# sholtodouglas/RoboticsPlayroomPybullet

Measured on AMD Instinct MI355X. Metric: env-steps/sec at N=4096 parallel UR5PlayAbsRPY1Obj-v0 envs per MI355X, higher is better.
Workload: dtype f32

## Files before the change

### roboticsplayroompybullet_amd/csrc/rp_kernels.cuh

```cuda
#pragma once
#include <hip/hip_runtime.h>
#include <stdint.h>

#include "rp_device_model.h"
#include "rp_math.cuh"

#define NB_MAX (1 + RP_MAX_ARM + RP_MAX_FREE + RP_MAX_J1)
#define NVP 28
#define MAXC 21
#define MAXACT 64
#define MAXT 4
#define MAXROWC (3 * MAXC + MAXT)
static_assert(MAXACT <= 64 && NB_MAX <= 32, "a candidate record packs its pair index in 6 bits and its bodies in 5 bits each");
#define PM_MAX 11
#define PMC_HDR 4
#define PMC_PT 11
#define PMC_MAN (8 + 4 * PMC_PT)
#define PMC_MANIFOLDS (PMC_HDR + PM_MAX * PMC_MAN)
#define PMC_AX PMC_MANIFOLDS
#define PMC_AXN 16
#define PMC_FLOATS (PMC_MANIFOLDS + 8 * PMC_AXN)
#define RP_MAX_GROUPS 16
#define SORT_KEYS 64
#define SORT_REPS 8
// ... 208 lines not shown
__device__ __forceinline__ int lane_pos(const DevModel* m, int d) {
  if (d < m->n_arm) return d;
  const int e = d - m->n_arm, f6 = 6 * m->n_free;
  if (e >= f6) return LANE_J1 + (e - f6);
  const int f = e / 6, c = e - 6 * f;
  return f == m->drawer_free ? m->n_arm + c : LANE_FREE + 6 * f + c;
}
__device__ __forceinline__ int lane_dof(const DevModel* m, int l) {
  if (l < m->n_arm) return l;
  if (l < 16) return l - m->n_arm < 6 ? m->n_arm + 6 * m->drawer_free + (l - m->n_arm) : -1;
  if (l >= 32) return -1;
  if (l < LANE_FREE) return l - LANE_J1 < m->n_j1 ? m->n_arm + 6 * m->n_free + (l - LANE_J1) : -1;
  return l - LANE_FREE < 12 ? m->n_arm + (l - LANE_FREE) : -1;
}
#endif
__device__ __forceinline__ float clampf(float v, float lo, float hi) { return fminf(fmaxf(v, lo), hi); }
__device__ __forceinline__ float safe_inv(float d) { return d > 1e-9f ? 1.0f / d : 0.0f; }
__device__ __forceinline__ int uni(int v) { return __builtin_amdgcn_readfirstlane(v); }
__device__ __forceinline__ float unif(float v) { return __int_as_float(__builtin_amdgcn_readfirstlane(__float_as_int(v))); }
__device__ __forceinline__ float lane_read(float v, int src_lane_uniform) {
  return __int_as_float(__builtin_amdgcn_readlane(__float_as_int(v), src_lane_uniform));
}

__device__ __forceinline__ double readlane_d(double v, int src_lane_uniform) {
  int lo = __builtin_amdgcn_readlane(__double2loint(v), src_lane_uniform), hi = __builtin_amdgcn_readlane(__double2hiint(v), src_lane_uniform);
  return __hiloint2double(hi, lo);
}

template <int K>
__device__ __forceinline__ float bcast16(float v) {
  return __int_as_float(__builtin_amdgcn_update_dpp(0, __float_as_int(v), 0x150 + (K & 15), 0xF, 0xF, true));
}
template <int T> struct IdxC { static constexpr int v = T; };
template <int I, int N, class F>
__device__ __forceinline__ void static_for(F&& f) {
  if constexpr (I < N) { f(IdxC<I>{}); static_for<I + 1, N>(f); }
}

template <int D>
__device__ __forceinline__ float shr16(float v) {
  return __int_as_float(__builtin_amdgcn_update_dpp(__float_as_int(v), __float_as_int(v), 0x110 + D, 0xF, 0xF, false));
}

__device__ __forceinline__ float wave_sum32(float v) {
  int x = __float_as_int(v);
  v += __int_as_float(__builtin_amdgcn_update_dpp(0, x, 0xB1, 0xF, 0xF, true));
  x = __float_as_int(v);
  v += __int_as_float(__builtin_amdgcn_update_dpp(0, x, 0x4E, 0xF, 0xF, true));
  x = __float_as_int(v);
  v += __int_as_float(__builtin_amdgcn_update_dpp(0, x, 0x141, 0xF, 0xF, true));
  x = __float_as_int(v);
  v += __int_as_float(__builtin_amdgcn_update_dpp(0, x, 0x140, 0xF, 0xF, true));
  return lane_read(v, 0) + lane_read(v, 16);
}

__device__ __forceinline__ uint64_t splitmix64(uint64_t x) {
  x += 0x9E3779B97F4A7C15ULL;
  x = (x ^ (x >> 30)) * 0xBF58476D1CE4E5B9ULL;
  x = (x ^ (x >> 27)) * 0x94D049BB133111EBULL;
  return x ^ (x >> 31);
}
__device__ __forceinline__ float rng_uniform(uint64_t seed, uint32_t env, uint32_t counter) {
  uint64_t h = splitmix64(seed ^ splitmix64(((uint64_t)env << 32) | counter));
  return (float)(h >> 40) * (1.0f / 16777216.0f);
}

struct Xf { M3 R; V3 p; };

__device__ __forceinline__ Xf joint_compose(const DevModel* m, const Xf& P, int j, float q) {
  Xf r;
  M3 Rj = mul(P.R, ldm3(m->arm_jrot[j]));
  r.p = P.p + mulv(P.R, ld3(m->arm_jpos[j]));
  V3 ax = ld3(m->arm_axis[j]);
  if (m->arm_jtype[j] == 0) {
    r.R = mul(Rj, axis_angle(ax, q));
  } else {
    r.R = Rj;
    r.p = r.p + mulv(Rj, ax) * q;
  }
  return r;
}

template <class LDS>
__device__ __forceinline__ void fk_bodies(const DevModel* m, LDS& L, int lane) {
  float* T = L.cand;
  static_assert(2 * 12 * RP_MAX_ARM + 2 * RP_MAX_ARM <= CANDMAX * 8 && 2 * 12 * RP_MAX_ARM + 2 * RP_MAX_ARM <= (int)(sizeof(L.cand) / sizeof(float)), "fk scratch fits the candidate list");
  int* P = (int*)(T + 2 * 12 * RP_MAX_ARM);
  const int n = m->n_arm;
  Xf x; x.R = ident3(); x.p = mk3(0, 0, 0);
  int par = -1;
  if (lane < n) {
    M3 R0 = ldm3(m->arm_jrot[lane]);
    V3 p0 = ld3(m->arm_jpos[lane]), ax = ld3(m->arm_axis[lane]);
    float q = L.st[ST_Q + lane];
    x.R = R0; x.p = p0;
    if (m->arm_jtype[lane] == 0) x.R = mul(R0, axis_angle(ax, q));
    else x.p = p0 + mulv(R0, ax) * q;
    par = m->arm_parent[lane];
    if (par < 0) { M3 Rb = ldm3(m->base_rot); V3 pb = ld3(m->base_pos); x.p = pb + mulv(Rb, x.p); x.R = mul(Rb, x.R); }
  }
  for (int it = 0; __ballot(par >= 0) != 0ull; it++) {
    float* Tb = T + (it & 1) * 12 * RP_MAX_ARM;
    int* Pb = P + (it & 1) * RP_MAX_ARM;
    if (lane < n) { stm3(&Tb[12 * lane], x.R); st3(&Tb[12 * lane + 9], x.p); Pb[lane] = par; }
    WSYNC();
    if (par >= 0) {
      M3 Ra = ldm3(&Tb[12 * par]); V3 pa = ld3(&Tb[12 * par + 9]);
      x.p = pa + mulv(Ra, x.p); x.R = mul(Ra, x.R);
      par = Pb[par];
    }
  }
  if (lane < n) { stm3(&L.xR[9 * (lane + 1)], x.R); st3(&L.xp[3 * (lane + 1)], x.p); }
  if (lane < m->nbody && !(lane >= 1 && lane <= n)) {
    int b = lane;
    Xf y; y.R = ident3(); y.p = mk3(0, 0, 0);
    if (b > n && b <= n + m->n_free) {
      int k = b - 1 - n;
      const float* f = &L.st[ST_FREE + 13 * k];
      Q4 q = {f[3], f[4], f[5], f[6]};
      y.R = quat_to_m3(q); y.p = ld3(f);
    } else if (b > n + m->n_free) {
      int k = b - 1 - n - m->n_free;
      M3 R0 = ldm3(m->j1_rot[k]);
      V3 ax = ld3(m->j1_axis[k]);
      y.p = ld3(m->j1_pos[k]);
      float q = L.st[ST_JQ + k];
      if (m->j1_type[k] == 0) y.R = mul(R0, axis_angle(ax, q));
      else { y.R = R0; y.p = y.p + mulv(R0, ax) * q; }
    }
    stm3(&L.xR[9 * b], y.R); st3(&L.xp[3 * b], y.p);
  }
}

template <class LDS>
__device__ __forceinline__ void joint_subspaces(const DevModel* m, LDS& L, int lane) {
  if (lane == 0) st3(L.O, ld3(&L.xp[3 * m->site_body[RP_SITE_EE]]));
  WSYNC();
  if (lane < m->n_arm) {
    V3 O = ld3(L.O);
    M3 R = ldm3(&L.xR[9 * (1 + lane)]);
    V3 a = mulv(R, ld3(m->arm_axis[lane]));
    V6 S;
    if (m->arm_jtype[lane] == 0) { S.a = a; S.l = cross(ld3(&L.xp[3 * (1 + lane)]) - O, a); }
    else { S.a = mk3(0, 0, 0); S.l = a; }
    st6(&L.S[6 * lane], S);
  }
}

template <class LDS>
__device__ __forceinline__ Xf collider_xf(const DevModel* m, const LDS& L, int c) {
  int b = m->col_body[c];
  M3 Rb = ldm3(&L.xR[9 * b]);
  Xf x;
  x.R = mul(Rb, ldm3(m->col_rot[c]));
  x.p = ld3(&L.xp[3 * b]) + mulv(Rb, ld3(m->col_pos[c]));
  return x;
}

template <class LDS>
__device__ __forceinline__ void collider_aabbs(const DevModel* m, LDS& L, int lane) {
  if (lane < m->n_col) {
    Xf x = collider_xf(m, L, lane);
    V3 he = ld3(m->col_he[lane]);
    float e[3];
    for (int i = 0; i < 3; i++)
      e[i] = m->col_type[lane] == 0 ? fabsf(x.R.m[3 * i]) * he.x + fabsf(x.R.m[3 * i + 1]) * he.y + fabsf(x.R.m[3 * i + 2]) * he.z : he.x;
    *(float4*)&L.aabb[8 * lane] = make_float4(x.p.x - e[0], x.p.y - e[1], x.p.z - e[2], m->col_margin[lane]);
    *(float4*)&L.aabb[8 * lane + 4] = make_float4(x.p.x + e[0], x.p.y + e[1], x.p.z + e[2], 0.f);
  }
}

struct CPt { V3 p, n; float dist; };

__device__ __forceinline__ int sphere_box(V3 cs, float r, V3 cb, const M3& Rb, V3 hb, float margin, int sphere_is_b, CPt* out) {
  const V3 l = tmulv(Rb, cs - cb);
  V3 cl = l;
  bool inside = true;
  if (cl.x > hb.x) { cl.x = hb.x; inside = false; }
  if (cl.x < -hb.x) { cl.x = -hb.x; inside = false; }
  if (cl.y > hb.y) { cl.y = hb.y; inside = false; }
  if (cl.y < -hb.y) { cl.y = -hb.y; inside = false; }
  if (cl.z > hb.z) { cl.z = hb.z; inside = false; }
  if (cl.z < -hb.z) { cl.z = -hb.z; inside = false; }
  V3 nl; float dist;
  if (!inside) {
    const V3 df = cl - l;
    const float len = norm(df);
    dist = len - r;
    if (dist > margin) return 0;
    nl = df * (1.f / len);
  } else {
    const float px = hb.x - fabsf(l.x), py = hb.y - fabsf(l.y), pz = hb.z - fabsf(l.z);
    int k0 = 0; float best = 1e30f;
    if (px < best) { best = px; k0 = 0; }
    if (py < best) { best = py; k0 = 1; }
    if (pz < best) { best = pz; k0 = 2; }
    const float lk = k0 == 0 ? l.x : (k0 == 1 ? l.y : l.z), hk = k0 == 0 ? hb.x : (k0 == 1 ? hb.y : hb.z);
    const float nk = lk > 0.f ? -1.f : 1.f, ck = lk > 0.f ? hk : -hk;
    nl = mk3(k0 == 0 ? nk : 0.f, k0 == 1 ? nk : 0.f, k0 == 2 ? nk : 0.f);
    cl = mk3(k0 == 0 ? ck : cl.x, k0 == 1 ? ck : cl.y, k0 == 2 ? ck : cl.z);
    dist = -best - r;
  }
  const V3 nw = mulv(Rb, nl), pw = mulv(Rb, cl) + cb;
  out[0].p = pw - nw * (0.5f * dist);
  out[0].n = sphere_is_b ? nw : -nw;
  out[0].dist = dist;
  return 1;
}

#define NPG 8
#define NPG_SCRATCH 96
__device__ __forceinline__ V3 pick3(int i, V3 a, V3 b, V3 c) { return i == 0 ? a : (i == 1 ? b : c); }
__device__ __forceinline__ float pick1(int i, float a, float b, float c) { return i == 0 ? a : (i == 1 ? b : c); }

// ... 1406 lines not shown
  WSYNC();
}

#define SR_UNIT 0
#define SR_J1 1
#define SR_GEAR 2
#define SR_LIMIT 3

template <class LDS>
__device__ __forceinline__ void put_srow(LDS& L, int r, int type, int dofA, float sign, float rhs, float dinv, float lo, float hi, int dofB) {
  float* s = &L.srow[8 * r];
  s[0] = __int_as_float(type); s[1] = __int_as_float(dofA); s[2] = sign; s[3] = rhs; s[4] = dinv; s[5] = lo; s[6] = hi;
  s[7] = __int_as_float(dofB);
}

template <class LDS>
__device__ __forceinline__ int build_small_rows(const DevModel* m, LDS& L, int lane) {
  int n = m->n_arm, nr = 0;
  if (lane < m->n_j1) {
    int d = dof_j1(m, lane);
    float minv = m->j1_minv[lane], dinv = 1.f / minv;
    float des = m->j1_has_pos_motor[lane] ? K_KP * (m->j1_motor_target[lane] - L.st[ST_JQ + lane]) / K_DT : 0.f;
    float mx = m->j1_motor_maximp[lane];
    put_srow(L, lane, SR_J1, d, minv, (des - L.vstar[d]) * dinv, dinv, -mx, mx, 0);
  }
  nr = m->n_j1;
  {
    int i = lane >> 1, side = lane & 1;
    bool on = false; float pen = 0.f;
    if (lane < 2 * n && m->arm_limited[i]) {
      float q = L.st[ST_Q + i];
      pen = side == 0 ? q - m->arm_lower[i] : m->arm_upper[i] - q;
      on = m->spec_limits ? !(pen > K_LIMIT_ACTIVATION) : !(pen > 0.f);
    }
    unsigned long long mask = __ballot(on);
    if (on) {
      int r = nr + __popcll(mask & ((1ull << lane) - 1ull));
      float sgn = side == 0 ? 1.f : -1.f;
      float dinv = 1.f / L.Minv[i * 12 + i];
      float relv = sgn * L.vstar[i], pos_err = 0.f, vel_err = -relv;
      if (pen > 0.f) vel_err -= pen / K_DT; else pos_err = -pen * (m->spec_limits ? K_ERP : K_ERP_LIMIT) / K_DT;
      put_srow(L, r, SR_LIMIT, i, sgn, (pos_err + vel_err) * dinv, dinv, 0.f, K_LIMIT_MAXIMP, 0);
    }
    nr += __popcll(mask);
  }
  if (lane < n) {
    float dinv = 1.f / L.Minv[lane * 12 + lane];
    float mode = L.st[ST_MMODE + lane];
    float des = mode != 0.f ? K_KP * (L.st[ST_MTARGET + lane] - L.st[ST_Q + lane]) / K_DT : 0.f;
    float mx = L.st[ST_MMAXIMP + lane];
    put_srow(L, nr + lane, SR_UNIT, lane, 1.f, (des - L.vstar[lane]) * dinv, dinv, -mx, mx, 0);
  }
  nr += n;
  if (m->arm_type == RP_ARM_PANDA) {
    if (lane == 0) {
      int a = m->d9p, b = m->d10p;
      float ratio = -1.f;
      float diag = L.Minv[a * 12 + a] + 2.f * ratio * L.Minv[a * 12 + b] + ratio * ratio * L.Minv[b * 12 + b];
      float dinv = safe_inv(diag);
      float relv = L.vstar[a] + ratio * L.vstar[b];
      float pos_err = -(L.st[ST_Q + a] + ratio * L.st[ST_Q + b]) * 0.1f / K_DT;
      put_srow(L, nr, SR_GEAR, a, ratio, (pos_err - relv) * dinv, dinv, -50.f * K_DT, 50.f * K_DT, b);
    }
    nr += 1;
  }
  return nr;
}

template <class LDS>
__device__ __forceinline__ int tors_list(const DevModel* m, LDS& L, int lane, int ncon) {
  bool head = false; float spin = 0.f;
  if (lane < ncon) {
    const int a = L.cona[lane], b = L.conb[lane];
    head = lane == 0 || L.cona[lane - 1] != a || L.conb[lane - 1] != b;
    spin = m->col_spin[a] * m->col_friction[b] + m->col_spin[b] * m->col_friction[a];
  }
  const unsigned long long mk = __ballot(head && spin > 0.f);
  const int t = __popcll(mk & ((1ull << lane) - 1ull));
  if (head && spin > 0.f && t < MAXT) { L.torc[t] = lane; L.tors[t] = spin; }
  const int nt = __popcll(mk);
  return nt < MAXT ? nt : MAXT;
}

template <class LDS>
__device__ __forceinline__ void contact_rows(const DevModel* m, LDS& L, int lane, int c0, int nc, int nt) {
  const int n = m->n_arm;
  const int nrows = 3 * nc + nt;
  V3 O = ld3(L.O);
  for (int r = lane; r < nrows; r += 64) {
    int ci, dir;
    if (r < nc) { ci = c0 + r; dir = 0; }
    else if (r < nc + nt) { ci = L.torc[r - nc]; dir = 3; }
    else { ci = c0 + ((r - nc - nt) >> 1); dir = 1 + ((r - nc - nt) & 1); }
    V3 nrm = ld3(&L.conn[3 * ci]);
    const V3 pmid = ld3(&L.conp[3 * ci]);
    const V3 half = nrm * (0.5f * L.cond[ci]);
    V3 d = nrm;
    const bool tors = dir == 3;
    if (dir == 1 || dir == 2) {
      V3 t1, t2;
      if (fabsf(nrm.z) > 0.7071067811865475244f) {
        float a = nrm.y * nrm.y + nrm.z * nrm.z, k = 1.f / sqrtf(a);
        t1 = mk3(0.f, -nrm.z * k, nrm.y * k);
        t2 = mk3(a * k, -nrm.x * t1.z, nrm.x * t1.y);
      } else {
        float a = nrm.x * nrm.x + nrm.y * nrm.y, k = 1.f / sqrtf(a);
        t1 = mk3(-nrm.y * k, nrm.x * k, 0.f);
        t2 = mk3(-nrm.z * t1.y, nrm.z * t1.x, a * k);
      }
      d = dir == 1 ? t1 : t2;
    }
    float* J = &L.J[r * ROWW];
    float* B = &L.B[r * ROWW];
    for (int k = 0; k < ROWW; k++) { J[k] = 0.f; B[k] = 0.f; }
    bool has_arm = false;
    float diag = 0.f, relv = 0.f;
    int off0 = 64, off1 = 64;
    int bodyA = m->col_body[L.cona[ci]], bodyB = m->col_body[L.conb[ci]];
    bool any_arm = (bodyA >= 1 && bodyA <= n) || (bodyB >= 1 && bodyB <= n);
    int nother = 0;
    float Jr[RP_MAX_ARM];
#pragma unroll
    for (int k = 0; k < RP_MAX_ARM; k++) Jr[k] = 0.f;
    for (int side = 0; side < 2; side++) {
      int body = side == 0 ? bodyA : bodyB;
      float sign = side == 0 ? 1.f : -1.f;
      if (body == 0) continue;
      const V3 p = side == 0 ? pmid + half : pmid - half;
      if (body <= n) {
        V6 f; f.a = tors ? d : cross(p - O, d); f.l = tors ? mk3(0, 0, 0) : d;
        uint32_t anc = m->arm_anc[body - 1];
#pragma unroll
        for (int k = 0; k < RP_MAX_ARM; k++) {
          const float v = sign * dot6(ld6(&L.S[6 * k]), f);
          Jr[k] = (k < n && ((anc >> k) & 1u)) ? Jr[k] + v : Jr[k];
        }
        has_arm = true;
        continue;
      }
      int base = (any_arm || nother == 1) ? 12 : 0;
      nother++;
      if (body <= n + m->n_free) {
        int k = body - 1 - n, dd = dof_free(m, k);
        V3 rr = p - ld3(&L.st[ST_FREE + 13 * k]);
        V3 rxn = tors ? d : cross(rr, d);
        float im = 1.f / m->free_mass[k];
        M3 Ii = ldm3(&L.finv[9 * k]);
        V3 w = mulv(Ii, rxn);
        const V3 dl = tors ? mk3(0, 0, 0) : d;
        float jl[3] = {sign * dl.x, sign * dl.y, sign * dl.z}, ja[3] = {sign * rxn.x, sign * rxn.y, sign * rxn.z};
        float ba[3] = {sign * w.x, sign * w.y, sign * w.z};
        for (int i = 0; i < 3; i++) {
          J[base + i] = jl[i]; B[base + i] = jl[i] * im; J[base + 3 + i] = ja[i]; B[base + 3 + i] = ba[i];
          diag += jl[i] * jl[i] * im + ja[i] * ba[i];
          relv += jl[i] * L.vstar[dd + i] + ja[i] * L.vstar[dd + 3 + i];
        }
        if (base == 0) off0 = dd; else off1 = dd;
      } else {
        int k = body - 1 - n - m->n_free, dd = dof_j1(m, k);
        M3 R = ldm3(&L.xR[9 * body]);
        V3 a = mulv(R, ld3(m->j1_axis[k]));
        float j = tors ? (m->j1_type[k] == 1 ? 0.f : sign * dot(a, d)) : (m->j1_type[k] == 1 ? sign * dot(d, a) : sign * dot(a, cross(p - ld3(m->j1_pos[k]), d)));
        float minv = m->j1_minv[k];
        J[base] = j; B[base] = j * minv;
        diag += j * j * minv; relv += j * L.vstar[dd];
        if (base == 0) off0 = dd; else off1 = dd;
      }
    }
    if (has_arm) {
      off0 = 0;
#pragma unroll
      for (int k = 0; k < RP_MAX_ARM; k++) if (k < n) J[k] = Jr[k];
    }
    float* s = &L.rowS[4 * r];
    s[0] = diag; s[1] = relv; s[2] = dir == 0 ? 0.f : (tors ? L.tors[r - nc] : L.conmu[ci]); s[3] = __int_as_float(dir == 0 ? 0 : ci);
    float* t = &L.rowT[4 * r];
    t[0] = __int_as_float(has_arm ? 1 : 0); t[1] = dir == 0 ? 1e10f : 0.f; t[2] = __int_as_float(off0); t[3] = __int_as_float(off1);
  }
  WSYNC();
  for (int e = lane; e < nrows * n; e += 64) {
    int r = e / n, i = e - r * n;
    if (__float_as_int(L.rowT[4 * r]) != 0) {
      const float* J = &L.J[r * ROWW];
      const float* Mi = &L.Minv[i * 12];
      float b = 0.f;
#pragma unroll
      for (int k = 0; k < RP_MAX_ARM; k++) { const float t = Mi[k] * J[k]; b = k < n ? b + t : b; }
      L.B[r * ROWW + i] = b;
    }
  }
  WSYNC();
  for (int r = lane; r < nrows; r += 64) {
    float* s = &L.rowS[4 * r];
    float* t = &L.rowT[4 * r];
    float diag = s[0], relv = s[1];
    if (__float_as_int(t[0]) != 0) {
      const float* J = &L.J[r * ROWW];
      const float* B = &L.B[r * ROWW];
#pragma unroll
      for (int i = 0; i < RP_MAX_ARM; i++) { const float jb = J[i] * B[i], jv = J[i] * L.vstar[i]; diag = i < n ? diag + jb : diag; relv = i < n ? relv + jv : relv; }
    }
    float dinv, rhs, cfmr = 0.f;
    if (r < nc) {
      const int ci = c0 + r;
      float cfm = 0.f, erp = K_ERP;
      float s0 = m->col_stiff[L.cona[ci]], s1 = m->col_stiff[L.conb[ci]];
      if (s0 > 0.f || s1 > 0.f) {
        float d0 = s0 > 0.f ? m->col_damp[L.cona[ci]] : 0.1f, d1 = s1 > 0.f ? m->col_damp[L.conb[ci]] : 0.1f;
        if (!(s0 > 0.f)) s0 = 1e18f;
        if (!(s1 > 0.f)) s1 = 1e18f;
        float ks = 1.f / (1.f / s0 + 1.f / s1), kd = d0 + d1;
        cfm = 1.f / (K_DT * (K_DT * ks + kd));
        erp = (K_DT * ks) / (K_DT * ks + kd);
      }
      dinv = safe_inv(diag + cfm);
      cfmr = cfm * dinv;
      float pen = L.cond[ci] + K_SLOP, pos_err = 0.f, vel_err = -relv;
      if (pen > 0.f) vel_err -= pen / K_DT; else pos_err = -pen * erp / K_DT;
      rhs = (pos_err + vel_err) * dinv;
    } else { dinv = safe_inv(diag); rhs = -relv * dinv; }
    s[0] = rhs; s[1] = cfmr;
    t[0] = __int_as_float((__float_as_int(t[0]) != 0 && __float_as_int(t[3]) != 64) ? 1 : 0);
    float* Jw = &L.J[r * ROWW];
    for (int k = 0; k < ROWW; k++) Jw[k] *= dinv;
  }
}

__device__ __forceinline__ float pgs_update(float delta, float lam, float lo, float hi, float& lam_out) {
  float d = __builtin_amdgcn_fmed3f(delta, lo - lam, hi - lam);
  lam_out = lam + d;
  return d;
}

template <class LDS>
__device__ float solve_rows(const DevModel* m, LDS& L, int lane, int nsmall_, int ncon_, int nt_) {
  const int n = m->n_arm;
  const int nsmall = uni(nsmall_), nrc = uni(3 * ncon_ + nt_);
  float dv = 0.f;
  float lamS = 0.f, lamC0 = 0.f, lamC1 = 0.f;
  for (int it = 0; it < K_NITER; it++) {
    {
      for (int rr = 0; rr < nsmall; rr++) {
        const int r = (it & 1) ? rr : nsmall - 1 - rr;
        const float4 c0 = *(const float4*)&L.srow[8 * r], c1 = *(const float4*)&L.srow[8 * r + 4];
        const int type_ = uni(__float_as_int(c0.x)), dA = uni(__float_as_int(c0.y)), dB = uni(__float_as_int(c1.w));
        const int type = type_ == SR_LIMIT ? SR_UNIT : type_;
        const float sg = c0.z, jA = c1.x;
        float bl = 0.f;
        if (type == SR_J1) bl = lane == lane_pos(m, dA) ? sg : 0.f;
        else if (lane < n) bl = type == SR_UNIT ? sg * L.Minv[lane * 12 + dA] : L.Minv[lane * 12 + dA] + sg * L.Minv[lane * 12 + dB];
        float delta;
        if (type == SR_UNIT) delta = __fmaf_rn(-(sg * jA), lane_read(dv, dA), c0.w);
        else if (type == SR_J1) delta = __fmaf_rn(-jA, lane_read(dv, uni(lane_pos(m, dA))), c0.w);
        else { float pa = jA * lane_read(dv, dA); float pb = (sg * jA) * lane_read(dv, dB); float jdv = pa + pb; delta = c0.w - jdv; }
        float lam = lane_read(lamS, r), lnew;
        const float d = pgs_update(delta, lam, c1.y, c1.z, lnew);
        lamS = lane == r ? lnew : lamS;
        dv = fmaf(bl, d, dv);
      }
    }
    if (nrc > 0) {
      float4 sn = *(const float4*)&L.rowS[0], tn = *(const float4*)&L.rowT[0];
      float4 s2 = sn, t2 = tn;
      if (nrc > 1) { s2 = *(const float4*)&L.rowS[4]; t2 = *(const float4*)&L.rowT[4]; }
      float jn = 0.f, bn = 0.f;
      const int mydof = lane_dof(m, lane);
      {
        int i1 = mydof - __float_as_int(tn.w), i0 = mydof - __float_as_int(tn.z);
        int idx = (unsigned)i1 < 6u ? 12 + i1 : ((unsigned)i0 < 12u ? i0 : -1);
        if (idx >= 0 && mydof >= 0) { jn = L.J[idx]; bn = L.B[idx]; }
      }
      for (int r = 0; r < nrc; r++) {
        float jl = jn, bl = bn;
        float rhs = sn.x, cfmr = sn.y, mu = sn.z, lo_c = 0.f, hi_c = tn.y;
        int parent = uni(__float_as_int(sn.w));
// ... 901 lines not shown
    else if (nc == 6) { for (int rep = 0; rep < 4; rep++) qj = ik_coop<6>(m, tpos, tq, qj, 20, l16, live, &ik_capped, &ik_marginal); }
    else { for (int rep = 0; rep < 4; rep++) qj = ik_coop<7>(m, tpos, tq, qj, 20, l16, live, &ik_capped, &ik_marginal); }
  }
  if (!live) return;
  if (l16 < nd) {
    float t = clampf(qj, m->ll[l16], m->ul[l16]);
    t = clampf(t, q0 - m->inc[l16], q0 + m->inc[l16]);
    st[ST_MMODE + l16] = 1.f; st[ST_MTARGET + l16] = t; st[ST_MMAXIMP + l16] = 240.f * K_DT;
    if (target_poses) target_poses[(size_t)env * nd + l16] = t;
  }
  if (l16 == 0) {
    st[ST_STATUS] = __int_as_float((ik_capped ? 8 : 0) | (ik_marginal ? 16 : 0));
    float g = a8[m->n_action - 1];
    if (m->arm_type == RP_ARM_PANDA) {
      float amt = 0.04f - g / 25.f;
      int ds[2] = {m->d9p, m->d10p};
      for (int i = 0; i < 2; i++) { st[ST_MMODE + ds[i]] = 1.f; st[ST_MTARGET + ds[i]] = amt; st[ST_MMAXIMP + ds[i]] = 100.f * K_DT; }
    } else {
      float amt = g - 0.2f;
      float left = st[ST_Q + m->d18];
      int ds[6] = {m->d18, m->d20, m->d12, m->d15, m->d10, m->d13};
      float tg[6] = {amt * 0.055f, left, amt * 0.5f, amt * 0.5f, amt * 0.8f, amt * 0.8f};
      float fo[6] = {100.f, 1000.f, 100.f, 100.f, 100.f, 100.f};
      for (int i = 0; i < 6; i++) { st[ST_MMODE + ds[i]] = 1.f; st[ST_MTARGET + ds[i]] = tg[i]; st[ST_MMAXIMP + ds[i]] = fo[i] * K_DT; }
    }
  }
}

__global__ void __launch_bounds__(64) k_action(const DevModel* __restrict__ m, float* __restrict__ state, const float* __restrict__ action,
                                              float* __restrict__ target_poses, int env0, int N, const int* __restrict__ member) {
  action_body(m, state, action, target_poses, env0, N, member, blockIdx.x);
}

__device__ __forceinline__ void copy_out(float* __restrict__ dst, const float* src, int nfloat, int lane) {
  for (int i = lane * 4; i < nfloat; i += 256) *(float4*)(dst + i) = *(const float4*)(src + i);
}

#define NBJ 3
#define LBL_N NBJ
#define NLBL (LBL_N + MAXC)
#define GEAR_LANE 12
#define W3_HDR 0
#define W3_VSTAR 8
#define W3_MU 40
#define W3_MINV 72
#define W3_A 216
#define W3_GEAR (W3_A + 160)
#define W3_ZERO (W3_GEAR + 7)
#define W3_BJ (W3_GEAR + 8)
#define W3_ROWS (W3_BJ + 20)
#define W3_ROWT (W3_ROWS + 4 * MAXROWC)
#define W3_ROFF (W3_ROWT + 4 * MAXROWC)
#define W3_SLOT (W3_ROFF + 64)
#define W3_J (W3_SLOT + 64)
#define W3_B (W3_J + ROWREG)
#define W3_SROW (W3_B + ROWREG)
#define W3_FLOATS (W3_SROW + 4 + 8 * MAXSMALL)
#define STAGE_FLOATS (128 + 2 * ROWREG)
#define AOUT_FLOATS (160 + 8 + 20)
static_assert(W3_A % 4 == 0 && W3_ROWS % 4 == 0 && W3_ROFF % 4 == 0 && AOUT_FLOATS % 4 == 0, "16-byte copies");

#define HV_MAXC 14
#ifndef S4_SLOTS0
#define S4_SLOTS0 8
#endif
#ifndef S4_SLOTS1
#define S4_SLOTS1 8
#endif
__device__ __forceinline__ int hv_class(int nc, int nA, int nB, int nC) {
  const bool heavy = nC != 0 || nA > S4_SLOTS0 || nB > S4_SLOTS1;
  return !heavy ? 0 : (nc <= HV_MAXC ? 1 : 2);
}
#define PREP_THREADS 128
__device__ __forceinline__ void prep2_core(PrepLds& L, const DevModel* __restrict__ m, const float* __restrict__ state, float* __restrict__ ws, const int env, const int cenv,
                                           int* __restrict__ pair_tab, const int pair_idx, int* __restrict__ hv_cnt = nullptr, int* __restrict__ hv_list = nullptr, const int prep_flags = 0) {
  const int tid = threadIdx.x, wid = tid >> 6, lane = tid & 63;
  PCLK(6) PCLK(0) PCLK_ZERO(15) PCLK_ZERO(19) PCLK_ZERO(26) PCLK_ZERO(27) PCLK_ZERO(28) PCLK_ZERO(29) PCLK_ZERO(30) PCLK_ZERO(31)
  static_assert(RP_REC_FLOATS == PREP_THREADS, "one float of the record per thread");
  L.st[tid] = state[(size_t)env * RP_REC_FLOATS + tid];
  if (tid == 64) L.hdr[3] = pair_idx;
  if (tid == 64 && m->persist) L.hdr[2] = __float_as_int(m->pmcache[(size_t)cenv * PMC_FLOATS]);
  __syncthreads();
  PCLK(16)
  if (wid == 0) fk_bodies(m, L, lane);
  __syncthreads();
  PCLK(17)
  float* w = ws + (size_t)env * W3_FLOATS;
  if (wid == 0) {
    collider_aabbs(m, L, lane);
    WSYNC();
    PCLK(1)
    int ncon = collide<PrepLds>(m, L, lane, cenv, &L.hdr[2]);
    ncon = uni(ncon);
#ifdef RP_ABL_MAXCON
    if (ncon > RP_ABL_MAXCON) ncon = RP_ABL_MAXCON;
#endif
    if (lane == 0) L.hdr[0] = ncon;
    PCLK(2)
  } else {
    joint_subspaces(m, L, lane);
    PCLK(18)
    arm_dynamics(m, L, lane);
    unconstrained_velocities(m, L, lane);
    PCLK(3)
    int nsmall = build_small_rows(m, L, lane);
    nsmall = uni(nsmall);
    for (int i = lane; i < AOUT_FLOATS; i += 64) L.aout[i] = 0.f;
    if (lane < 2) L.amask[lane] = 0u;
    if (lane == 2) L.amask[2] = (unsigned)nsmall;
    WSYNC();
    bool gear = false;
    if (lane < nsmall) {
      const float* s = &L.srow[8 * lane];
      int type = __float_as_int(s[0]), dA = __float_as_int(s[1]);
      float sg = s[2], rhs = s[3], dinv = s[4], lo = s[5], hi = s[6];
      if (type == SR_UNIT) {
        L.aout[dA] = dinv; L.aout[16 + dA] = rhs; L.aout[32 + dA] = lo; L.aout[48 + dA] = hi;
      } else if (type == SR_LIMIT) {
        int pl = sg > 0.f ? 64 : 112;
        L.aout[pl + dA] = sg * rhs; L.aout[pl + 16 + dA] = sg * lo; L.aout[pl + 32 + dA] = sg * hi;
        atomicOr(&L.amask[sg > 0.f ? 0 : 1], 1u << dA);
      } else if (type == SR_J1) {
        int k = lane;
        if (k < NBJ) { float* bq = &L.aout[168]; bq[k] = dinv; bq[4 + k] = rhs; bq[8 + k] = lo; bq[12 + k] = hi; bq[16 + k] = sg; }
      } else {
        float* g = &L.aout[160];
        g[0] = s[1]; g[1] = s[7]; g[2] = sg; g[3] = dinv; g[4] = rhs; g[5] = lo; g[6] = hi;
        gear = true;
      }
    }
    const bool anygear = __ballot(gear) != 0ull;
    if (lane == 0) L.hdr[1] = anygear ? 1 : 0;
    WSYNC();
    if (lane < 32) w[W3_VSTAR + lane] = L.vstar[lane];
    copy_out(w + W3_MINV, L.Minv, 144, lane);
    copy_out(w + W3_A, L.aout, AOUT_FLOATS, lane);
  }
  __syncthreads();
  const int ncon = L.hdr[0];
  int tid_j = threadIdx.x;
  asm volatile("" : "+v"(tid_j));
  const int wid_j = tid_j >> 6;
  if (wid_j == 0) {
    const int lane = tid_j & 63;
    float* w = ws + (size_t)env * W3_FLOATS;
    const int cls = lane < ncon ? L.conk[lane] : 3;
    const unsigned long long mB = __ballot(cls == 0), mA = __ballot(cls == 1), mC = __ballot(cls == 2);
    const unsigned long long lower = (1ull << lane) - 1ull;
    L.slot[lane] = -1;
    L.roff[lane] = 0;
    const int nt = tors_list(m, L, lane, ncon);
    WSYNC();
    if (cls == 0) L.slot[__popcll(mB & lower)] = lane;
    else if (cls == 1) L.slot[21 + __popcll(mA & lower)] = lane;
    else if (cls == 2) L.slot[42 + __popcll(mC & lower)] = lane;
    bool tors_done = nt == 0;
    for (int c0 = 0; c0 < ncon || !tors_done; c0 += PREP_CH) {
      const int nc = max(0, min(PREP_CH, ncon - c0));
      const int ntl = (!tors_done && c0 + PREP_CH >= ncon && 3 * nc + nt <= 3 * PREP_CH) ? nt : 0;
      contact_rows(m, L, lane, c0, nc, ntl);
      WSYNC();
      auto global_row = [&](int lr) { return lr < nc ? c0 + lr : (lr < nc + ntl ? 3 * ncon + (lr - nc) : ncon + 2 * c0 + (lr - nc - ntl)); };
      for (int e = lane; e < (3 * nc + ntl) * ROWW; e += 64) {
        const int lr = e / ROWW, k = e - lr * ROWW;
        const int gr = global_row(lr);
        w[W3_J + gr * ROWW + k] = L.J[e]; w[W3_B + gr * ROWW + k] = L.B[e];
      }
      for (int e = lane; e < (3 * nc + ntl) * 4; e += 64) {
        const int lr = e >> 2, k = e & 3;
        const int gr = global_row(lr);
        float v = L.rowS[e];
        if (k == 3 && lr >= nc && lr < nc + ntl) {
          const int c = L.torc[lr - nc], kc = L.conk[c];
          const unsigned long long mk = kc == 1 ? mA : (kc == 2 ? mC : mB);
          v = __int_as_float(c | (kc << 8) | (__popcll(mk & ((1ull << c) - 1ull)) << 12));
        }
        w[W3_ROWS + gr * 4 + k] = v; w[W3_ROWT + gr * 4 + k] = L.rowT[e];
      }
      if (lane < 3 * nc + ntl && !(lane >= nc && lane < nc + ntl)) {
        const int gr = global_row(lane);
        L.roff[gr] = __float_as_int(L.rowT[4 * lane + 2]) | (__float_as_int(L.rowT[4 * lane + 3]) << 8);
      }
      if (ntl > 0) tors_done = true;
      WSYNC();
    }
    PCLK(4)
    if (lane == 0) {
      int nj = m->n_j1 < NBJ ? m->n_j1 : NBJ;
      w[W3_HDR] = __int_as_float((int)L.amask[0]); w[W3_HDR + 1] = __int_as_float((int)L.amask[1]);
      w[W3_HDR + 2] = __int_as_float(nj); w[W3_HDR + 3] = __int_as_float(ncon);
      w[W3_HDR + 4] = __int_as_float(__popcll(mA)); w[W3_HDR + 5] = __int_as_float(__popcll(mB));
      w[W3_HDR + 6] = __int_as_float(L.hdr[1] | (nt << 8)); w[W3_HDR + 7] = __int_as_float(__popcll(mC));
      if (hv_list != nullptr && (hv_class(ncon, __popcll(mA), __popcll(mB), __popcll(mC)) != 0 || (prep_flags & 1))) hv_list[atomicAdd(hv_cnt, 1)] = env | (ncon << 24);
    }
    if (lane < 32) w[W3_MU + lane] = lane < ncon ? L.conmu[lane] : 0.f;
    copy_out(w + W3_ROFF, (const float*)L.roff, 64, lane);
    copy_out(w + W3_SLOT, (const float*)L.slot, 64, lane);
  } else {
    if ((tid_j & 63) == 0) pair_tab[L.hdr[3]] = env | (ncon << 24);
    if (prep_flags & 1) {
      const int lane = tid_j & 63;
      float* w = ws + (size_t)env * W3_FLOATS;
      const int nsm = (int)L.amask[2];
      if (lane == 0) w[W3_SROW] = __int_as_float(nsm);
      for (int i = lane; i < 8 * nsm; i += 64) w[W3_SROW + 4 + i] = L.srow[i];
    }
  }
  PCLK(5) PCLK(7)
}
__device__ __forceinline__ void prep2_body(const DevModel* __restrict__ m, const float* __restrict__ state, float* __restrict__ ws, int env0, int N,
                                           const int* __restrict__ sort_cnt, int* __restrict__ sort_cnt_next, const int* __restrict__ sort_slot, int* __restrict__ pair_env,
                                           const int* __restrict__ member, const int bid, const int* __restrict__ cache_env = nullptr, int* __restrict__ hv_cnt = nullptr, int* __restrict__ hv_cnt_next = nullptr,
                                           int* __restrict__ hv_list = nullptr, const int prep_flags = 0) {
  __shared__ PrepLds L;
  const int tid = threadIdx.x, wid = tid >> 6, lane = tid & 63;
  int env = env0 + bid;
  if (env >= N) return;
  if (member) env = member[env];
  if (bid == 0) {
    for (int i = tid; i < SORT_BINS; i += PREP_THREADS) sort_cnt_next[i] = 0;
    if (tid == 0 && hv_cnt_next) *hv_cnt_next = 0;
  }
  int pair_place = 0;
  if (wid == 1) {
    const int my_slot = sort_slot[env];
    int cnt8[8];
#pragma unroll
    for (int t = 0; t < 8; t++) cnt8[t] = sort_cnt[8 * lane + t];
    const int mybin = my_slot >> SORT_RANK_BITS;
    int above = 0;
#pragma unroll
    for (int t = 0; t < 8; t++) above += (8 * lane + t > mybin) ? cnt8[t] : 0;
#pragma unroll
    for (int d = 32; d >= 1; d >>= 1) above += __shfl_xor(above, d);
    pair_place = above + (my_slot & SORT_RANK_MASK);
  }
  prep2_core(L, m, state, ws, env, cache_env ? cache_env[env] : env, pair_env, env0 + pair_place, hv_cnt, hv_list ? hv_list + env0 : nullptr, prep_flags);
}
#define PREP2_ARGS const DevModel* __restrict__ m, const float* __restrict__ state, float* __restrict__ ws, int env0, int N, \
                   const int* __restrict__ sort_cnt, int* __restrict__ sort_cnt_next, const int* __restrict__ sort_slot, int* __restrict__ pair_env, \
                   const int* __restrict__ member
#define HV_ARGS int* __restrict__ hv_cnt, int* __restrict__ hv_cnt_next, int* __restrict__ hv_list, int prep_flags
__global__ void __launch_bounds__(PREP_THREADS, RP_PREP_WAVES) k_prep2(PREP2_ARGS, HV_ARGS) { prep2_body(m, state, ws, env0, N, sort_cnt, sort_cnt_next, sort_slot, pair_env, member, blockIdx.x, nullptr, hv_cnt, hv_cnt_next, hv_list, prep_flags); }
__global__ void __launch_bounds__(PREP_THREADS, RP_PREP_WAVES) k_settle_prep(PREP2_ARGS, const int* __restrict__ cache_env, int prep_flags) { prep2_body(m, state, ws, env0, N, sort_cnt, sort_cnt_next, sort_slot, pair_env, member, blockIdx.x, cache_env, nullptr, nullptr, nullptr, prep_flags); }
__global__ void __launch_bounds__(PREP_THREADS, RP_PREP_WAVES) k_action_prep(const DevModel* __restrict__ m, float* __restrict__ state, float* __restrict__ ws, int env0, int N,
                                                                   const int* __restrict__ sort_cnt, int* __restrict__ sort_cnt_next, const int* __restrict__ sort_slot,
                                                                   int* __restrict__ pair_env, const int* __restrict__ member, const float* __restrict__ action,
                                                                   float* __restrict__ target_poses, int nab, HV_ARGS) {
  if ((int)blockIdx.x < nab) {
    __builtin_amdgcn_s_setprio(3);
    action_body(m, state, action, target_poses, env0, N, member, blockIdx.x);
  }
  else prep2_body(m, state, ws, env0, N, sort_cnt, sort_cnt_next, sort_slot, pair_env, member, blockIdx.x - nab, nullptr, hv_cnt, hv_cnt_next, hv_list, prep_flags);
}


typedef float f16v __attribute__((ext_vector_type(16)));
__device__ __forceinline__ float row16_sum(float v) {
  int x = __float_as_int(v);
  v += __int_as_float(__builtin_amdgcn_update_dpp(0, x, 0xB1, 0xF, 0xF, true));
  x = __float_as_int(v);
  v += __int_as_float(__builtin_amdgcn_update_dpp(0, x, 0x4E, 0xF, 0xF, true));
  x = __float_as_int(v);
  v += __int_as_float(__builtin_amdgcn_update_dpp(0, x, 0x141, 0xF, 0xF, true));
  x = __float_as_int(v);
  v += __int_as_float(__builtin_amdgcn_update_dpp(0, x, 0x140, 0xF, 0xF, true));
  return v;
}
__device__ __forceinline__ float fold_rows(float v) {
  unsigned u = __float_as_uint(v);
  auto sw = __builtin_amdgcn_permlane16_swap(u, u, false, false);
  return __uint_as_float(sw[0]) + __uint_as_float(sw[1]);
}
struct Plane { float rhs, lo, hi, lam, dacc, loP, hiP; };
struct PlaneN : Plane { float cfm, rhsE; };
#define PLANE_FENCE4(a, b, c, d) asm volatile("s_nop 1" : "+v"((a).loP), "+v"((a).hiP), "+v"((b).loP), "+v"((b).hiP), "+v"((c).loP), "+v"((c).hiP), "+v"((d).loP), "+v"((d).hiP))
#define PLANE_FENCE_N(a, b, c) asm volatile("s_nop 1" : "+v"((a).loP), "+v"((a).hiP), "+v"((b).rhsE), "+v"((c).rhsE))
__device__ __forceinline__ void plane_begin(Plane& p) { p.loP = p.lo - p.lam; p.hiP = p.hi - p.lam; p.dacc = 0.f; }
__device__ __forceinline__ void plane_end(Plane& p) { p.lam += p.dacc; }
__device__ __forceinline__ void nplane_begin(PlaneN& p) { p.loP = p.lo - p.lam; p.hiP = p.hi - p.lam; p.dacc = 0.f; p.rhsE = __fmaf_rn(-p.lam, p.cfm, p.rhs); }
__device__ __forceinline__ void fplane_begin(Plane& p, float lim, float tot) {
  const bool on = tot > 0.f;
  p.loP = on ? (0.f - lim) - p.lam : 0.f; p.hiP = on ? (0.f + lim) - p.lam : 0.f; p.dacc = 0.f;
}

#define DPP_ALL " row_mask:0xf bank_mask:0xf bound_ctrl:1\n"

template <int I>
// ... 1466 lines not shown
```

Measured before the change: 2.136 million.

## Spread contact-row build and body FK across all block wavefronts

The prep kernel's contact Jacobian row construction, previously run by wavefront 0 alone while other waves idled, now runs across all PREP_THREADS threads, with block-wide barriers in place of wave syncs. Forward kinematics is split so wave 0 handles the arm chain while the other waves compute free and single-joint bodies at the same time. This aims to shorten the serial critical path per environment, at the cost of more __syncthreads barriers and a shared torsion count passed through LDS.

```diff
diff --git a/roboticsplayroompybullet_amd/csrc/rp_kernels.cuh b/roboticsplayroompybullet_amd/csrc/rp_kernels.cuh
--- a/roboticsplayroompybullet_amd/csrc/rp_kernels.cuh
+++ b/roboticsplayroompybullet_amd/csrc/rp_kernels.cuh
@@ -314,7 +314,7 @@
 }
 
 template <class LDS>
-__device__ __forceinline__ void fk_bodies(const DevModel* m, LDS& L, int lane) {
+__device__ __forceinline__ void fk_arm_links(const DevModel* m, LDS& L, int lane) {
   float* T = L.cand;
   static_assert(2 * 12 * RP_MAX_ARM + 2 * RP_MAX_ARM <= CANDMAX * 8 && 2 * 12 * RP_MAX_ARM + 2 * RP_MAX_ARM <= (int)(sizeof(L.cand) / sizeof(float)), "fk scratch fits the candidate list");
   int* P = (int*)(T + 2 * 12 * RP_MAX_ARM);
@@ -343,6 +343,10 @@
     }
   }
   if (lane < n) { stm3(&L.xR[9 * (lane + 1)], x.R); st3(&L.xp[3 * (lane + 1)], x.p); }
+}
+template <class LDS>
+__device__ __forceinline__ void fk_other_bodies(const DevModel* m, LDS& L, int lane) {
+  const int n = m->n_arm;
   if (lane < m->nbody && !(lane >= 1 && lane <= n)) {
     int b = lane;
     Xf y; y.R = ident3(); y.p = mk3(0, 0, 0);
@@ -362,6 +366,11 @@
     }
     stm3(&L.xR[9 * b], y.R); st3(&L.xp[3 * b], y.p);
   }
+}
+template <class LDS>
+__device__ __forceinline__ void fk_bodies(const DevModel* m, LDS& L, int lane) {
+  fk_arm_links(m, L, lane);
+  fk_other_bodies(m, L, lane);
 }
 
 template <class LDS>
@@ -1934,12 +1943,16 @@
   return nt < MAXT ? nt : MAXT;
 }
 
-template <class LDS>
+template <int NTHR>
+__device__ __forceinline__ void rows_sync() {
+  if constexpr (NTHR == 64) WSYNC(); else __syncthreads();
+}
+template <class LDS, int NTHR = 64>
 __device__ __forceinline__ void contact_rows(const DevModel* m, LDS& L, int lane, int c0, int nc, int nt) {
   const int n = m->n_arm;
   const int nrows = 3 * nc + nt;
   V3 O = ld3(L.O);
-  for (int r = lane; r < nrows; r += 64) {
+  for (int r = lane; r < nrows; r += NTHR) {
     int ci, dir;
     if (r < nc) { ci = c0 + r; dir = 0; }
     else if (r < nc + nt) { ci = L.torc[r - nc]; dir = 3; }
@@ -2029,8 +2042,8 @@
     float* t = &L.rowT[4 * r];
     t[0] = __int_as_float(has_arm ? 1 : 0); t[1] = dir == 0 ? 1e10f : 0.f; t[2] = __int_as_float(off0); t[3] = __int_as_float(off1);
   }
-  WSYNC();
-  for (int e = lane; e < nrows * n; e += 64) {
+  rows_sync<NTHR>();
+  for (int e = lane; e < nrows * n; e += NTHR) {
     int r = e / n, i = e - r * n;
     if (__float_as_int(L.rowT[4 * r]) != 0) {
       const float* J = &L.J[r * ROWW];
@@ -2041,8 +2054,8 @@
       L.B[r * ROWW + i] = b;
     }
   }
-  WSYNC();
-  for (int r = lane; r < nrows; r += 64) {
+  rows_sync<NTHR>();
+  for (int r = lane; r < nrows; r += NTHR) {
     float* s = &L.rowS[4 * r];
     float* t = &L.rowT[4 * r];
     float diag = s[0], relv = s[1];
@@ -3110,7 +3123,8 @@
   if (tid == 64 && m->persist) L.hdr[2] = __float_as_int(m->pmcache[(size_t)cenv * PMC_FLOATS]);
   __syncthreads();
   PCLK(16)
-  if (wid == 0) fk_bodies(m, L, lane);
+  if (wid == 0) fk_arm_links(m, L, lane);
+  else fk_other_bodies(m, L, lane);
   __syncthreads();
   PCLK(17)
   float* w = ws + (size_t)env * W3_FLOATS;
@@ -3168,70 +3182,72 @@
   const int ncon = L.hdr[0];
   int tid_j = threadIdx.x;
   asm volatile("" : "+v"(tid_j));
-  const int wid_j = tid_j >> 6;
+  const int wid_j = tid_j >> 6, lane_j = tid_j & 63;
+  float* wr = ws + (size_t)env * W3_FLOATS;
+  const int cls = lane_j < ncon ? L.conk[lane_j] : 3;
+  const unsigned long long mB = __ballot(cls == 0), mA = __ballot(cls == 1), mC = __ballot(cls == 2);
   if (wid_j == 0) {
-    const int lane = tid_j & 63;
-    float* w = ws + (size_t)env * W3_FLOATS;
-    const int cls = lane < ncon ? L.conk[lane] : 3;
-    const unsigned long long mB = __ballot(cls == 0), mA = __ballot(cls == 1), mC = __ballot(cls == 2);
-    const unsigned long long lower = (1ull << lane) - 1ull;
-    L.slot[lane] = -1;
-    L.roff[lane] = 0;
-    const int nt = tors_list(m, L, lane, ncon);
+    const unsigned long long lower = (1ull << lane_j) - 1ull;
+    L.slot[lane_j] = -1;
+    L.roff[lane_j] = 0;
+    const int nt = tors_list(m, L, lane_j, ncon);
+    if (lane_j == 0) L.hdr[2] = nt;
     WSYNC();
-    if (cls == 0) L.slot[__popcll(mB & lower)] = lane;
-    else if (cls == 1) L.slot[21 + __popcll(mA & lower)] = lane;
-    else if (cls == 2) L.slot[42 + __popcll(mC & lower)] = lane;
-    bool tors_done = nt == 0;
-    for (int c0 = 0; c0 < ncon || !tors_done; c0 += PREP_CH) {
-      const int nc = max(0, min(PREP_CH, ncon - c0));
-      const int ntl = (!tors_done && c0 + PREP_CH >= ncon && 3 * nc + nt <= 3 * PREP_CH) ? nt : 0;
-      contact_rows(m, L, lane, c0, nc, ntl);
-      WSYNC();
-      auto global_row = [&](int lr) { return lr < nc ? c0 + lr : (lr < nc + ntl ? 3 * ncon + (lr - nc) : ncon + 2 * c0 + (lr - nc - ntl)); };
-      for (int e = lane; e < (3 * nc + ntl) * ROWW; e += 64) {
-        const int lr = e / ROWW, k = e - lr * ROWW;
-        const int gr = global_row(lr);
-        w[W3_J + gr * ROWW + k] = L.J[e]; w[W3_B + gr * ROWW + k] = L.B[e];
-      }
-      for (int e = lane; e < (3 * nc + ntl) * 4; e += 64) {
-        const int lr = e >> 2, k = e & 3;
-        const int gr = global_row(lr);
-        float v = L.rowS[e];
-        if (k == 3 && lr >= nc && lr < nc + ntl) {
-          const int c = L.torc[lr - nc], kc = L.conk[c];
-          const unsigned long long mk = kc == 1 ? mA : (kc == 2 ? mC : mB);
-          v = __int_as_float(c | (kc << 8) | (__popcll(mk & ((1ull << c) - 1ull)) << 12));
-        }
-        w[W3_ROWS + gr * 4 + k] = v; w[W3_ROWT + gr * 4 + k] = L.rowT[e];
-      }
-      if (lane < 3 * nc + ntl && !(lane >= nc && lane < nc + ntl)) {
-        const int gr = global_row(lane);
-        L.roff[gr] = __float_as_int(L.rowT[4 * lane + 2]) | (__float_as_int(L.rowT[4 * lane + 3]) << 8);
-      }
-      if (ntl > 0) tors_done = true;
-      WSYNC();
-    }
-    PCLK(4)
-    if (lane == 0) {
+    if (cls == 0) L.slot[__popcll(mB & lower)] = lane_j;
+    else if (cls == 1) L.slot[21 + __popcll(mA & lower)] = lane_j;
+    else if (cls == 2) L.slot[42 + __popcll(mC & lower)] = lane_j;
+  }
+  __syncthreads();
+  const int nt = uni(L.hdr[2]);
+  bool tors_done = nt == 0;
+  for (int c0 = 0; c0 < ncon || !tors_done; c0 += PREP_CH) {
+    const int nc = max(0, min(PREP_CH, ncon - c0));
+    const int ntl = (!tors_done && c0 + PREP_CH >= ncon && 3 * nc + nt <= 3 * PREP_CH) ? nt : 0;
+    contact_rows<PrepLds, PREP_THREADS>(m, L, tid_j, c0, nc, ntl);
+    __syncthreads();
+    auto global_row = [&](int lr) { return lr < nc ? c0 + lr : (lr < nc + ntl ? 3 * ncon + (lr - nc) : ncon + 2 * c0 + (lr - nc - ntl)); };
+    for (int e = tid_j; e < (3 * nc + ntl) * ROWW; e += PREP_THREADS) {
+      const int lr = e / ROWW, k = e - lr * ROWW;
+      const int gr = global_row(lr);
+      wr[W3_J + gr * ROWW + k] = L.J[e]; wr[W3_B + gr * ROWW + k] = L.B[e];
+    }
+    for (int e = tid_j; e < (3 * nc + ntl) * 4; e += PREP_THREADS) {
+      const int lr = e >> 2, k = e & 3;
+      const int gr = global_row(lr);
+      float v = L.rowS[e];
+      if (k == 3 && lr >= nc && lr < nc + ntl) {
+        const int c = L.torc[lr - nc], kc = L.conk[c];
+        const unsigned long long mk = kc == 1 ? mA : (kc == 2 ? mC : mB);
+        v = __int_as_float(c | (kc << 8) | (__popcll(mk & ((1ull << c) - 1ull)) << 12));
+      }
+      wr[W3_ROWS + gr * 4 + k] = v; wr[W3_ROWT + gr * 4 + k] = L.rowT[e];
+    }
+    if (tid_j < 3 * nc + ntl && !(tid_j >= nc && tid_j < nc + ntl)) {
+      const int gr = global_row(tid_j);
+      L.roff[gr] = __float_as_int(L.rowT[4 * tid_j + 2]) | (__float_as_int(L.rowT[4 * tid_j + 3]) << 8);
+    }
+    if (ntl > 0) tors_done = true;
+    __syncthreads();
+  }
+  PCLK(4)
+  if (wid_j == 0) {
+    if (lane_j == 0) {
       int nj = m->n_j1 < NBJ ? m->n_j1 : NBJ;
-      w[W3_HDR] = __int_as_float((int)L.amask[0]); w[W3_HDR + 1] = __int_as_float((int)L.amask[1]);
-      w[W3_HDR + 2] = __int_as_float(nj); w[W3_HDR + 3] = __int_as_float(ncon);
-      w[W3_HDR + 4] = __int_as_float(__popcll(mA)); w[W3_HDR + 5] = __int_as_float(__popcll(mB));
-      w[W3_HDR + 6] = __int_as_float(L.hdr[1] | (nt << 8)); w[W3_HDR + 7] = __int_as_float(__popcll(mC));
+      wr[W3_HDR] = __int_as_float((int)L.amask[0]); wr[W3_HDR + 1] = __int_as_float((int)L.amask[1]);
+      wr[W3_HDR + 2] = __int_as_float(nj); wr[W3_HDR + 3] = __int_as_float(ncon);
+      wr[W3_HDR + 4] = __int_as_float(__popcll(mA)); wr[W3_HDR + 5] = __int_as_float(__popcll(mB));
+      wr[W3_HDR + 6] = __int_as_float(L.hdr[1] | (nt << 8)); wr[W3_HDR + 7] = __int_as_float(__popcll(mC));
       if (hv_list != nullptr && (hv_class(ncon, __popcll(mA), __popcll(mB), __popcll(mC)) != 0 || (prep_flags & 1))) hv_list[atomicAdd(hv_cnt, 1)] = env | (ncon << 24);
     }
-    if (lane < 32) w[W3_MU + lane] = lane < ncon ? L.conmu[lane] : 0.f;
-    copy_out(w + W3_ROFF, (const float*)L.roff, 64, lane);
-    copy_out(w + W3_SLOT, (const float*)L.slot, 64, lane);
+    if (lane_j < 32) wr[W3_MU + lane_j] = lane_j < ncon ? L.conmu[lane_j] : 0.f;
+    copy_out(wr + W3_ROFF, (const float*)L.roff, 64, lane_j);
   } else {
-    if ((tid_j & 63) == 0) pair_tab[L.hdr[3]] = env | (ncon << 24);
+    copy_out(wr + W3_SLOT, (const float*)L.slot, 64, lane_j);
+    if (lane_j == 0) pair_tab[L.hdr[3]] = env | (ncon << 24);
     if (prep_flags & 1) {
-      const int lane = tid_j & 63;
-      float* w = ws + (size_t)env * W3_FLOATS;
       const int nsm = (int)L.amask[2];
-      if (lane == 0) w[W3_SROW] = __int_as_float(nsm);
-      for (int i = lane; i < 8 * nsm; i += 64) w[W3_SROW + 4 + i] = L.srow[i];
+      if (lane_j == 0) wr[W3_SROW] = __int_as_float(nsm);
+      for (int i = lane_j; i < 8 * nsm; i += 64) wr[W3_SROW + 4 + i] = L.srow[i];
     }
   }
   PCLK(5) PCLK(7)
```

Result: no change. 2.156 million (median of 6 runs) (+1.0%).
